# liron88/HM-16.2

Measured on AMD Instinct MI355X. Metric: CTUs/sec (enc) at 4K main10; bit-exact CU partition vs HM, higher is better.
Workload: dtype int32+f64

## Files before the change

__graft_entry__.py:

```python
import os
import subprocess
import sys

ROOT = os.path.dirname(os.path.abspath(__file__))
PKG = os.path.join(ROOT, "hm-16.2_amd")
for p in (ROOT, PKG, os.path.join(ROOT, "oracle")):
    if p not in sys.path:
        sys.path.insert(0, p)


def _newer(target, sources):
    if not os.path.exists(target):
        return True
    t = os.path.getmtime(target)
    return any(os.path.getmtime(s) > t for s in sources)


def build_product():
    src = os.path.join(PKG, "csrc")
    out = os.path.join(PKG, "libhm355.so")
    deps = [os.path.join(src, f) for f in ("hm355.hip", "hm355_core.h", "hm355_inter.h", "hm355_inter_cu.h", "hm355_dbk.h", "hm355_sao.h", "hm355_bits.h", "hm355_bits_kernel.h", "hm355_ingest.h", "hm355_picstat.h", "hm355_types.h", "hm355_host_common.h", "hm355_simt.h", "hm355_simt4.h", "hm355_simt8.h", "hm355_simt16.h", "hm355_team.h")] + [os.path.join(ROOT, "include", "hm355.h")]
    if _newer(out, deps):
        import hashlib
        h = hashlib.sha1()
        for d in sorted(deps):
            h.update(open(d, "rb").read())
        build_id = h.hexdigest()[:12]
        hipcc = "/opt/rocm/bin/hipcc" if os.path.exists("/opt/rocm/bin/hipcc") else "hipcc"
        cmd = [hipcc, "-O3", "--offload-arch=gfx950", "-ffp-contract=off", "-fPIC", "-shared", "-std=c++17", "-Wno-unused-value", "-Wno-sizeof-array-div",
               f'-DHM355_BUILD_ID="{build_id}"', "-o", out, os.path.join(src, "hm355.hip")]
        subprocess.run(cmd, check=True)
    host = os.path.join(PKG, "host")
    exe = os.path.join(PKG, "hm355_encmain")
    if _newer(exe, [os.path.join(host, f) for f in ("encmain.cpp", "TEncTop.cpp", "TEncTop.h")] + [out]):
        subprocess.run(["g++", "-O2", "-std=c++14", "-Wall", "-o", exe, os.path.join(host, "encmain.cpp"), os.path.join(host, "TEncTop.cpp"),
                        "-L" + PKG, "-lhm355", "-Wl,-rpath,$ORIGIN"], check=True)
    return out


def build_oracle():
    subprocess.run(["make", "-s", "-C", os.path.join(ROOT, "oracle"),
                    os.path.join(ROOT, "oracle", "libhm_oracle.so"), os.path.join(ROOT, "oracle", "hm_oracle_cli")], check=True)
    if os.path.isdir("/root/reference/source"):
        subprocess.run(["make", "-s", "-C", os.path.join(ROOT, "oracle"), "ref"], check=True, stdout=subprocess.DEVNULL)


def build():
    build_product()
    build_oracle()
    import hm355
    hm355.load_library()


def smoke():
# ... 59 lines not shown
```

hm-16.2_amd/csrc/hm355_core.h:

```cpp
#pragma once
#include <stddef.h>
#include "hm355_types.h"

#ifdef HM355_HOSTSIM
#include <string.h>
#include <math.h>
#include <stdlib.h>
#define HM_DEV static
#define HM_FINL static inline
#define HM_FINL_M inline
#define HM_LAMBDA_INL
#define HM_NOINLINE __attribute__((noinline))
#define HM_CONST static const
#define HM_ASSUME_LDS(p) ((void)0)
#define HM_ASSUME_GLB(p) ((void)0)
#define HM_NT 1
static inline int hm_lane() { return 0; }
#define HM_SYNC() ((void)0)
static inline uint32_t hm_wave_sum(uint32_t v) { return v; }
static inline int hm_wave_sum_i(int v) { return v; }
static inline int hm_wave_max_i(int v) { return v; }
#define HM_UNI(x) (x)
#define HM_UCALL(x) (x)
#define hm_uni_ptr(p) (p)
// ... 65 lines not shown
{
  static_assert(sizeof(T) % 4 == 0, "dword-sized aggregates only");
  int w[sizeof(T) / 4];
  __builtin_memcpy(w, &v, sizeof(T));
#pragma unroll
  for (unsigned i = 0; i < sizeof(T) / 4; i++) w[i] = __builtin_amdgcn_readfirstlane(w[i]);
  __builtin_memcpy(&v, w, sizeof(T));
  return v;
}
#define HM_ENTRY(e) do { (e) = hm_uni_ptr(e); HM_ASSUME_LDS(e); } while (0)
#define HM_UCALL(x) ((uint32_t)__builtin_amdgcn_readfirstlane((int)(x)))
#define HM_PAR_FOR(i, n) for (int i = hm_lane(); i < (n); i += HM_NT)
#define HM_PAR_FOR_XY(x, y, w, n) \
  for (int i_ = hm_lane(), sy_ = HM_NT / (w), sx_ = HM_NT - sy_ * (w), y = i_ / (w), x = i_ - y * (w); i_ < (n); \
       i_ += HM_NT, x += sx_, y += sy_, (x >= (w) ? (x -= (w), y++) : 0))
#define HM_WAVE_FOR(k) for (int k = hm_lane(), k##_once = 1; k##_once; k##_once = 0)
#define HM_LV(T, name) T name
#define HM_LVARG(T, name) const T name
#define HM_LVK(name, k) name
#define HM_LV_GET(name, i) __builtin_amdgcn_readlane((int)(name), (int)(i))
#define HM_LV_GETD(name, i) hm_readlane_d((name), (int)(i))
#define HM_LV_SET(name, i, v) ((name) = (hm_lane() == (int)(i)) ? (v) : (name))
#define HM_LV_SETD(name, i, v) ((name) = (hm_lane() == (int)(i)) ? (v) : (name))
#define HM_LV_GATHER(name, idx) __builtin_amdgcn_ds_bpermute((int)(idx) << 2, (int)(name))
#define HM_BALLOT(m, k, cond) ((m) = __ballot(cond))
#define HM_ORDERED_ADD16(acc, name) do { _Pragma("unroll") for (int k_ = 15; k_ >= 0; k_--) (acc) += hm_readlane_d((name), k_); } while (0)
#define HM_ORDERED_CHAIN16(acc, a, b, pre) do { _Pragma("unroll") for (int k_ = 15; k_ >= 0; k_--) { \
    (pre) = (hm_lane() == k_) ? (acc) : (pre); (acc) -= hm_readlane_d((a), k_); (acc) += hm_readlane_d((b), k_); } } while (0)
__device__ __forceinline__ double hm_readlane_d(double v, int i)
{ return __hiloint2double(__builtin_amdgcn_readlane(__double2hiint(v), i), __builtin_amdgcn_readlane(__double2loint(v), i)); }
#endif

#if defined(HM355_PROFILE) && !defined(HM355_HOSTSIM)
#define HM_PROF_N 45
#define HM_PROF_BEGIN(e, id) const unsigned long long prof_t0_##id = __builtin_readcyclecounter()
#define HM_PROF_END(e, id) do { (e)->prof[id] += __builtin_readcyclecounter() - prof_t0_##id; (e)->profCnt[id] += 1; } while (0)
#else
#define HM_PROF_BEGIN(e, id) ((void)0)
#define HM_PROF_END(e, id) ((void)0)
#endif
enum { PR_RDOQ = 0, PR_BITS, PR_ADI, PR_PRED, PR_FWD, PR_INV, PR_SATD35, PR_TUBLK, PR_SAVE, PR_CHROMA, PR_LUMA, PR_ENCCU, PR_TOTAL,
       PR_S4L = 32, PR_S4C, PR_D0, PR_D1, PR_D2, PR_D3, PR_NXN, PR_S8L, PR_S4LEAF, PR_S4CLEAF, PR_S8C, PR_S16L = 44,
       PR_ME_INT = 16, PR_ME_FRAC, PR_AMVP, PR_MRG_EST, PR_MC, PR_IRQ, PR_IRES, PR_MRG2N, PR_INTERCU, PR_INTRA_IN_P, PR_IQ_FULL, PR_IQ_FWD, PR_IQ_RDOQ, PR_IQ_BITS, PR_IQ_INV, PR_IQ_ENC };

#define HM_MAX_DOUBLE 1.7e+308
#define PLANAR_IDX 0
#define DC_IDX 1
#define HOR_IDX 10
#define VER_IDX 26
#define DM_CHROMA_IDX 36
#define SIZE_2Nx2N 0
#define SIZE_NxN 3
#define SIZE_NONE 8
#define MODE_INTRA 1
#define MODE_NONE 2
#define SCAN_DIAG 0
#define SCAN_HOR 1
#define SCAN_VER 2

HM_CONST uint8_t HM_NEXT_LPS[128] __attribute__((aligned(4))) = {
  1, 0, 0, 1, 2, 3, 4, 5, 4, 5, 8, 9, 8, 9, 10, 11, 12, 13, 14, 15, 16, 17, 18, 19, 18, 19, 22, 23, 22, 23, 24, 25,
  26, 27, 26, 27, 30, 31, 30, 31, 32, 33, 32, 33, 36, 37, 36, 37, 38, 39, 38, 39, 42, 43, 42, 43, 44, 45, 44, 45, 46, 47, 48, 49,
  48, 49, 50, 51, 52, 53, 52, 53, 54, 55, 54, 55, 56, 57, 58, 59, 58, 59, 60, 61, 60, 61, 60, 61, 62, 63, 64, 65, 64, 65, 66, 67,
  66, 67, 66, 67, 68, 69, 68, 69, 70, 71, 70, 71, 70, 71, 72, 73, 72, 73, 72, 73, 74, 75, 74, 75, 74, 75, 76, 77, 76, 77, 126, 127 };
HM_CONST int32_t HM_ENTROPY_BITS[128] = {
  0x07b23, 0x085f9, 0x074a0, 0x08cbc, 0x06ee4, 0x09354, 0x067f4, 0x09c1b, 0x060b0, 0x0a62a, 0x05a9c, 0x0af5b, 0x0548d, 0x0b955, 0x04f56, 0x0c2a9,
  0x04a87, 0x0cbf7, 0x045d6, 0x0d5c3, 0x04144, 0x0e01b, 0x03d88, 0x0e937, 0x039e0, 0x0f2cd, 0x03663, 0x0fc9e, 0x03347, 0x10600, 0x03050, 0x10f95,
  0x02d4d, 0x11a02, 0x02ad3, 0x12333, 0x0286e, 0x12cad, 0x02604, 0x136df, 0x02425, 0x13f48, 0x021f4, 0x149c4, 0x0203e, 0x1527b, 0x01e4d, 0x15d00,
  0x01c99, 0x166de, 0x01b18, 0x17017, 0x019a5, 0x17988, 0x01841, 0x18327, 0x016df, 0x18d50, 0x015d9, 0x19547, 0x0147c, 0x1a083, 0x0138e, 0x1a8a3,
  0x01251, 0x1b418, 0x01166, 0x1bd27, 0x01068, 0x1c77b, 0x00f7f, 0x1d18e, 0x00eda, 0x1d91a, 0x00e19, 0x1e254, 0x00d4f, 0x1ec9a, 0x00c90, 0x1f6e0,
  0x00c01, 0x1fef8, 0x00b5f, 0x208b1, 0x00ab6, 0x21362, 0x00a15, 0x21e46, 0x00988, 0x2285d, 0x00934, 0x22ea8, 0x008a8, 0x239b2, 0x0081d, 0x24577,
  0x007c9, 0x24ce6, 0x00763, 0x25663, 0x00710, 0x25e8f, 0x006a0, 0x26a26, 0x00672, 0x26f23, 0x005e8, 0x27ef8, 0x005ba, 0x284b5, 0x0055e, 0x29057,
  0x0050c, 0x29bab, 0x004c1, 0x2a674, 0x004a7, 0x2aa5e, 0x0046f, 0x2b32f, 0x0041f, 0x2c0ad, 0x003e7, 0x2ca8d, 0x003ba, 0x2d323, 0x0010c, 0x3bfbb };
HM_CONST uint8_t HM_CTX_INIT_I[HM_NUM_CTX] = {
   139, 141, 157,
// ... 1754 lines not shown
        cabac_copy(&e->cur, &e->ws->slot[HM_SLOT(fullDepth, CI_QT_TRAFO_ROOT)]);
        const uint32_t splitBits = HM_UCALL(intra_bits_qt(e, *t, 1, 0));
        f->splitCost = calc_rd_cost(e, splitBits, f->splitDist);
        if (f->splitCost < f->singleCost) { retDist[sp] += f->splitDist; retBits[sp] += splitBits; retCost[sp] += f->splitCost; sp--; continue; }
      }
      cabac_copy(&e->cur, &e->ws->slot[HM_SLOT(fullDepth, CI_QT_TRAFO_TEST)]);
      par_set8(m->tr + z, t->trDepth, t->parts);
      par_set8(m->cbf[0] + z, (int)(f->singleCbf << t->trDepth), t->parts);
      par_set8(m->ts[0] + z, f->bestModeId, t->parts);
      {
        const int n = 1 << log2, layer = 5 - log2, ps = e->stride[0];
        par_copy_blk(e->fb.rec[0] + (e->ctuY * 64 + t->y) * ps + e->ctuX * 64 + t->x, ps, e->ws->qtRec[layer] + t->y * 64 + t->x, 64, n);
      }
      retDist[sp] += f->singleDist; retBits[sp] += f->singleBits; retCost[sp] += f->singleCost; sp--; continue;
    }
  }
  e->outDistY = retDist[0]; e->outRdCost = retCost[0];
}

HM_DEV inline void set_intra_result_qt(Shared *e, const TU *root)
{
  const CtuMeta *m = (&e->meta);
  for (int rel = root->relZ; rel < root->relZ + root->parts;) {
    const int z = root->cuZ + rel, trd = m->tr[z];
    const int log2 = 6 - root->cuDepth - trd, n = 1 << log2, layer = 5 - log2;
    const int parts = root->cuParts >> (2 * trd) > 0 ? root->cuParts >> (2 * trd) : 1;
    const int r = hm_z2r(z), x = (r & 15) * 4, y = (r >> 4) * 4;
    par_copy32(e->cc + z * 16, e->ws->qtCoef[layer] + z * 16, n * n);
    par_copy_blk(e->ws->reco + y * 64 + x, 64, e->ws->qtRec[layer] + y * 64 + x, 64, n);
    rel += parts;
  }
}

#include "hm355_simt.h"
#include "hm355_simt4.h"
#include "hm355_simt8.h"
#include "hm355_simt16.h"

HM_DEV HM_NOINLINE uint32_t est_intra_pred_qt(Shared *e, int cuZ, int cuDepth)
{
  HM_ENTRY(e); cuZ = HM_UNI(cuZ); cuDepth = HM_UNI(cuDepth);
  CtuMeta *m = (&e->meta); WorkSpace *ws = e->ws;
  const int cuParts = 256 >> (2 * cuDepth);
  const int nxn = m->part[cuZ] == SIZE_NxN;
  const int numPU = nxn ? 4 : 1, puParts = cuParts / numPU;
  const int puLog2 = 6 - cuDepth - nxn, n = 1 << puLog2;
  const int bitDepth = e->bitDepth, ps = e->stride[0];
  uint32_t overallDistY = 0;
  const TU root = tu_root(e, cuZ, cuDepth);
  for (int pu = 0; pu < numPU; pu++) {
    const TU t = nxn ? tu_child(&root, pu, 0) : root;
    const int z = cuZ + t.relZ;
    int numModesForFullRD = HM_INTRA_MODE_NUM_FAST[puLog2 - 1];
    int32_t *rdModeList = e->rdModeList;
    {
      const int r = hm_z2r(z);
      init_adi_pattern(e, 0, e->ctuX * 64 + t.x, e->ctuY * 64 + t.y, n, e->ctuX * 16 + (r & 15), e->ctuY * 16 + (r >> 4), n / 4, 1);
      const Pel *org = e->fb.org[0] + (e->ctuY * 64 + t.y) * ps + e->ctuX * 64 + t.x;
      Pel *pred = ws->pred + t.y * 64 + t.x;
      int preds[3];
      const int numMpm = intra_dir_predictor(e, z, preds);
      e->mpmZ = z; e->mpmNum = numMpm; e->mpmPreds[0] = preds[0]; e->mpmPreds[1] = preds[1]; e->mpmPreds[2] = preds[2];
      const uint64_t frac0 = e->ws->slot[HM_SLOT(cuDepth, CI_CURR_BEST)].frac & 32767;
      const uint8_t st0 = e->ws->slot[HM_SLOT(cuDepth, CI_CURR_BEST)].s[C_INTRA_LUMA];
      HM_PROF_BEGIN(e, PR_SATD35);
      if (n <= 16) satd_all_modes_small(e, org, ps, n);
      else {
        for (int mode = 0; mode < 35; mode++) {
          pred_intra(e, 0, mode, n, use_filtered_refs(0, mode, n), pred, 64);
          const uint32_t sad = dist_hads(org, ps, pred, 64, n, bitDepth);
// ... 106 lines not shown
      const int isOne = (total == 1), isLast = (currModeId == total);
      const uint32_t distTmp = HM_UCALL(intra_coding_tu_block(e, *t, comp, isOne ? 0 : (tsMode == 0 ? 1 : 2)));
      const uint32_t cbfTmp = (m->cbf[comp][zc] >> t->trDepth) & 1;
      if (tsMode == 1 && cbfTmp == 0) costTmp = HM_MAX_DOUBLE;
      else if (!isOne) { reset_bits(&e->cur); enc_coeff_qt(e, t, comp); costTmp = calc_rd_cost(e, num_bits(&e->cur), distTmp); }
      if (costTmp < singleCost) {
        singleCost = costTmp; singleDistC = distTmp; bestTS = tsMode; bestModeId = currModeId; singleCbfC = cbfTmp;
        if (!isOne && !isLast) { store_intra_result_qt(e, t, comp); cabac_copy(&e->ws->slot[HM_SLOT(fullDepth, CI_TEMP_BEST)], &e->cur); }
      }
      if (!isOne && !isLast) cabac_copy(&e->cur, &e->ws->slot[HM_SLOT(fullDepth, CI_QT_TRAFO_ROOT)]);
    }
    if (bestModeId < total) {
      load_intra_result_qt(e, t, comp);
      par_set8(m->cbf[comp] + zc, (int)(singleCbfC << t->trDepth), t->cParts);
      cabac_copy(&e->cur, &e->ws->slot[HM_SLOT(fullDepth, CI_TEMP_BEST)]);
    }
    par_set8(m->ts[comp] + zc, bestTS, t->cParts);
    dist += singleDistC;
  }
  return dist;
}
HM_DEV HM_NOINLINE uint32_t recur_intra_chroma_coding_qt(Shared *e, TU rootv)
{
  HM_ENTRY(e); rootv = hm_uni_struct(rootv);
  const TU *root = &rootv;
  CtuMeta *m = (&e->meta);
  uint32_t dist = 0;
  tu_walk(e->walkOuter, root, 0,
    [&](const TU *t) {
      if (m->tr[t->cuZ + t->relZ] != t->trDepth) return 1;
      if (t->cW) dist += chroma_tu(e, t);
      return 0;
    },
    [&](const TU *t) {
      const int z = t->cuZ + t->relZ, q = t->parts >> 2;
      int any = 0;
      for (int c = 1; c < 3; c++) for (int s = 0; s < 4; s++) any |= ((m->cbf[c][z + s * q] >> (t->trDepth + 1)) & 1) << c;
      HM_PAR_FOR(o, t->parts) for (int c = 1; c < 3; c++) if ((any >> c) & 1) m->cbf[c][z + o] |= (uint8_t)(1 << t->trDepth);
      HM_SYNC();
    });
  return dist;
}
HM_DEV inline void set_intra_result_chroma_qt(Shared *e, const TU *root)
{
  const CtuMeta *m = (&e->meta);
  tu_walk(e->walkOuter, root, 0, [&](const TU *t) {
    if (!t->cW) return 0;
    if (m->tr[t->cuZ + t->relZ] != t->trDepth) return 1;
    const int n = t->cW, layer = 5 - t->log2;
    for (int c = 1; c < 3; c++) {
      const int po = HM_PLANE_OFF(c);
      par_copy32(e->cc + po + t->cOff, e->ws->qtCoef[layer] + po + t->cOff, n * n);
      par_copy_blk(e->ws->reco + po + t->cy * 32 + t->cx, 32, e->ws->qtRec[layer] + po + t->cy * 32 + t->cx, 32, n);
    }
    return 0;
  });
}
HM_DEV HM_NOINLINE uint32_t est_intra_pred_chroma_qt(Shared *e, int cuZ, int cuDepth)
{
  HM_ENTRY(e); cuZ = HM_UNI(cuZ); cuDepth = HM_UNI(cuDepth);
  CtuMeta *m = (&e->meta); WorkSpace *ws = e->ws; const int cuParts = 256 >> (2 * cuDepth);
  const TU t = tu_root(e, cuZ, cuDepth);
  if (cuDepth == 3) {
    const int split = m->tr[cuZ] != 0;
    int tsLuma = 0;
    if (split) for (int s = 0; s < 4; s++) tsLuma += m->ts[0][cuZ + s];
    if (!tsLuma) {
      cabac_copy(&e->cur, &e->ws->slot[HM_SLOT(cuDepth, CI_CURR_BEST)]);
      HM_PROF_BEGIN(e, PR_S4C);
      const uint32_t d = HM_UCALL(simt4_chroma_cu(e, split ? tu_child(&t, 0, 0) : t, cuZ));
      HM_PROF_END(e, PR_S4C);
      cabac_copy(&e->cur, &e->ws->slot[HM_SLOT(cuDepth, CI_CURR_BEST)]);
      return d;
    }
  }
  if (cuDepth == 2) {
    int split = 0;
    for (int i = 0; i < 16; i += 4) split |= m->tr[cuZ + i];
    if (!split) {
      cabac_copy(&e->cur, &e->ws->slot[HM_SLOT(cuDepth, CI_CURR_BEST)]);
      HM_PROF_BEGIN(e, PR_S8C);
      const uint32_t d = HM_UCALL(simt8_chroma_cu16(e, cuZ));
      HM_PROF_END(e, PR_S8C);
      cabac_copy(&e->cur, &e->ws->slot[HM_SLOT(cuDepth, CI_CURR_BEST)]);
      return d;
    }
  }
  int bestMode = 0; uint32_t bestDist = 0; double bestCost = HM_MAX_DOUBLE;
  int modeList[5];
  allowed_chroma_dirs(m->dirL[cuZ], modeList);
  for (int mi = 0; mi < 5; mi++) {
    cabac_copy(&e->cur, &e->ws->slot[HM_SLOT(cuDepth, CI_CURR_BEST)]);
    par_set8(m->dirC + cuZ, modeList[mi], cuParts);
    const uint32_t dist = HM_UCALL(recur_intra_chroma_coding_qt(e, t));
    cabac_copy(&e->cur, &e->ws->slot[HM_SLOT(cuDepth, CI_CURR_BEST)]);
    const uint32_t bits = HM_UCALL(intra_bits_qt(e, t, 0, 1));
    const double cost = calc_rd_cost(e, bits, dist);
    if (cost < bestCost) {
      bestCost = cost; bestDist = dist; bestMode = modeList[mi];
      set_intra_result_chroma_qt(e, &t);
      HM_PAR_FOR(i, cuParts) for (int c = 1; c < 3; c++) { ws->saveCbf[c][i] = m->cbf[c][cuZ + i]; ws->saveTs[c][i] = m->ts[c][cuZ + i]; }
      HM_SYNC();
    }
  }
  HM_PAR_FOR(i, cuParts) { for (int c = 1; c < 3; c++) { m->cbf[c][cuZ + i] = ws->saveCbf[c][i]; m->ts[c][cuZ + i] = ws->saveTs[c][i]; } m->dirC[cuZ + i] = (uint8_t)bestMode; }
  HM_SYNC();
  cabac_copy(&e->cur, &e->ws->slot[HM_SLOT(cuDepth, CI_CURR_BEST)]);
  return bestDist;
}

template <class C> HM_DEV inline void code_delta_qp(Shared *e, C *c, int dqp)
{
  const int off = 6 * (e->bitDepth - 8);
  dqp = (dqp + 78 + off + (off / 2)) % (52 + off) - 26 - (off / 2);
  const uint32_t a = (uint32_t)hm_abs(dqp), tu = a < 5 ? a : 5;
  enc_bin(e, c, C_DQP, tu ? 1 : 0);
  if (tu) { for (uint32_t k = tu; --k;) enc_bin(e, c, C_DQP + 1, 1); if (5 > tu) enc_bin(e, c, C_DQP + 1, 0); }
  if (a >= 5) {
    uint32_t sym = a - 5, count = 0, bins = 0; int nb = 0;
    while (sym >= (1u << count)) { bins = 2 * bins + 1; nb++; sym -= 1u << count; count++; }
    bins = 2 * bins; nb++;
    bins = (bins << count) | sym; nb += (int)count;
    enc_epv(c, bins, nb);
  }
  if (a > 0) enc_epv(c, dqp > 0 ? 0u : 1u, 1);
}
template <class C> HM_DEV inline void code_dqp_if_due(Shared *e, C *c)
{
  if (!e->fb.dqp) return;
  WorkSpace *ws = e->ws;
  if (!HM_UNI(ws->dq.flag)) return;
  code_delta_qp(e, c, HM_UNI(ws->dq.ctuQp) - HM_UNI(ws->dq.refQp));
  HM_SYNC();
  if (hm_lane() == 0) ws->dq.flag = 0;
  HM_SYNC();
}
HM_DEV inline void check_dqp(Shared *e, int cuZ, int cuDepth)
{
  if (!e->fb.dqp || cuDepth != 0) return;
  const CtuMeta *m = &e->meta;
// ... 379 lines not shown
```

hm-16.2_amd/csrc/hm355_simt.h:

```cpp
#pragma once

template <int L2> struct SimtDim {
  enum { NC = 1 << (2 * L2), NCG = NC / 16, WCG = 1 << (L2 - 2), NSIG = L2 == 2 ? 9 : (L2 == 3 ? 21 : 27), NSET = NCG == 1 ? 1 : 4, NGRP = 2 * L2, NCGC = NCG == 1 ? 0 : 2,
         NLAST = L2 == 4 ? 4 : 3, LSH = L2 == 4 ? 1 : L2 - 2,
         X_SIG = 0, X_ONE = NSIG, X_ABS = X_ONE + 4 * NSET, X_LX = X_ABS + NSET, X_LY = X_LX + NLAST, X_CG = X_LY + NLAST, X_CBF = X_CG + NCGC,
         X_MODE = X_CBF + 1, X_TSKIP = X_MODE + 1, NCTX = X_TSKIP + (L2 == 2 ? 1 : 0),
         T_SIG = 0, T_ONE = 2 * NSIG, T_ABS = T_ONE + 8 * NSET, T_LASTX = T_ABS + 2 * NSET, T_LASTY = T_LASTX + NGRP, T_CG = T_LASTY + NGRP,
         T_CBF = T_CG + 2 * NCGC, T_N = T_CBF + 2 };
};
static_assert(SimtDim<2>::NCTX == 23 && SimtDim<2>::T_N == 38 && SimtDim<2>::X_LX == 14 && SimtDim<2>::X_LY == 17 && SimtDim<2>::X_CBF == 20 && SimtDim<2>::T_LASTX == 28 &&
              SimtDim<2>::T_LASTY == 32 && SimtDim<2>::T_CBF == 36 && SimtDim<2>::LSH == 0, "the 4x4 batch's numbering");
static_assert(SimtDim<3>::NCTX == 51 && SimtDim<3>::T_N == 100 && SimtDim<3>::X_ONE == 21 && SimtDim<3>::X_ABS == 37 && SimtDim<3>::X_LX == 41 && SimtDim<3>::X_LY == 44 &&
              SimtDim<3>::X_CG == 47 && SimtDim<3>::X_CBF == 49 && SimtDim<3>::T_ONE == 42 && SimtDim<3>::T_ABS == 74 && SimtDim<3>::T_LASTX == 82 && SimtDim<3>::T_LASTY == 88 &&
              SimtDim<3>::T_CG == 94 && SimtDim<3>::T_CBF == 98 && SimtDim<3>::LSH == 1 && SimtDim<3>::WCG == 2, "the 8x8 batch's numbering");
template <int L2> struct Simt;
template <int L2> struct SimtPrices {
  const int32_t *tab;
  HM_FINL_M int one(int i) const { return tab[SimtDim<L2>::T_ONE + i]; }
  HM_FINL_M int abs2(int i) const { return tab[SimtDim<L2>::T_ABS + i]; }
};

struct SimtPar {
  int chroma, bitDepth, qBits, quantCoef, tshift; double errScale, lambda; int64_t rdFactor;
  int dqShift, dqScale, dqMin, dqMax;
// ... 8 lines not shown
  int tgt = 25 + p.dqShift; if (tgt > 16) tgt = 16;
  p.dqMin = -(1 << (tgt - 1)); p.dqMax = (1 << (tgt - 1)) - 1;
  return p;
}
HM_FINL int32_t simt_level_double(int sc, const SimtPar &p)
{
  const int64_t cap = 2147483647LL - (1LL << (p.qBits - 1));
  const int64_t tl = (int64_t)hm_abs(sc) * p.quantCoef;
  return (int32_t)(tl < cap ? tl : cap);
}
HM_FINL int simt_dequant(const SimtPar &p, int level)
{
  const int c = hm_clip3(p.dqMin, p.dqMax, level);
  int v;
  if (p.dqShift > 0) v = (c * p.dqScale + (1 << (p.dqShift - 1))) >> p.dqShift;
  else v = (int)((unsigned)(c * p.dqScale) << (-p.dqShift));
  return hm_clip3(-32768, 32767, v);
}

template <int L2> HM_FINL int simt_ctx_index(int j, int chroma, int cbfCodeCtx, int modeCtx)
{
  typedef SimtDim<L2> D;
  const int lastOff = chroma ? 15 : 3 * (L2 - 2);
  if (j < D::X_ONE) return C_SIG + (chroma ? 28 : 0) + (chroma && j >= 16 ? 0 : j);
  if (j < D::X_ABS) return C_ONE + (chroma ? 16 + ((j - D::X_ONE) & 7) : j - D::X_ONE);
  if (j < D::X_LX) return C_ABS + (chroma ? 4 + ((j - D::X_ABS) & 1) : j - D::X_ABS);
  if (j < D::X_LY) return C_LASTX + lastOff + (j - D::X_LX);
  if (j < D::X_CG) return C_LASTY + lastOff + (j - D::X_LY);
  if (j < D::X_CBF) return C_SIG_CG + (chroma ? 2 : 0) + (j - D::X_CG);
  if (j == D::X_CBF) return C_QT_CBF + cbfCodeCtx;
  if (j == D::X_MODE) return modeCtx;
  return C_TSKIP + (chroma ? 1 : 0);
}
template <int L2> HM_DEV inline void simt_setup(Shared *e, const Simt<L2> &S, const Cabac *cb, int jobs, int chroma, int cbfCtx, int cbfCodeCtx, int modeCtx)
{
  typedef SimtDim<L2> D;
  HM_PAR_FOR(i, D::T_N) {
    const int bin = i & 1;
    int v = 0;
    if (i < D::T_LASTX) {
      const int j = i >> 1, none = chroma && ((j < D::X_ONE && j >= 16) || (j >= D::X_ONE && j < D::X_ABS && j - D::X_ONE >= 8) || (j >= D::X_ABS && j - D::X_ABS >= 2));
      if (!none) v = HM_LT()->ebits[cb->s[simt_ctx_index<L2>(j, chroma, 0, 0)] ^ bin];
    } else if (i < D::T_CG) {
      const int g = (i - D::T_LASTX) % D::NGRP, x0 = i < D::T_LASTY ? D::X_LX : D::X_LY;
      for (int c = 0; c < g; c++) v += HM_LT()->ebits[cb->s[simt_ctx_index<L2>(x0 + (c >> D::LSH), chroma, 0, 0)] ^ 1];
      if (g < D::NGRP - 1) v += HM_LT()->ebits[cb->s[simt_ctx_index<L2>(x0 + (g >> D::LSH), chroma, 0, 0)] ^ 0];
      if (g > 3) v += 32768 * ((g - 2) >> 1);
    } else if (i < D::T_CBF) v = HM_LT()->ebits[cb->s[simt_ctx_index<L2>(D::X_CG + ((i - D::T_CG) >> 1), chroma, 0, 0)] ^ bin];
    else v = HM_LT()->ebits[cb->s[C_QT_CBF + cbfCtx] ^ bin];
    S.tab()[i] = v;
  }
  HM_PAR_FOR(i, 128) S.lps()[i] = HM_NEXT_LPS[i];
  HM_PAR_FOR(i, D::NCTX * S.JOBS) {
    const int j = i / S.JOBS, k = i - j * S.JOBS;
    if (k < jobs) S.ctx(j, k) = cb->s[simt_ctx_index<L2>(j, chroma, cbfCodeCtx, modeCtx)];
  }
  S.load_scans(e);
  HM_SYNC();
}
template <int L2> HM_FINL void simt_store_contexts(const Simt<L2> &S, int k, Cabac *cb, int cbfCodeCtx)
{
  HM_PAR_FOR(j, SimtDim<L2>::NCTX) cb->s[simt_ctx_index<L2>(j, 0, cbfCodeCtx, C_INTRA_LUMA)] = S.ctx(j, k);
}

template <int L2> HM_DEV inline void simt_bin(const Shared *e, const Simt<L2> &S, int k, uint32_t *frac, int c, int bin)
{
  const int st = S.ctx(c, k);
  *frac += (uint32_t)HM_LT()->ebits[st ^ bin];
  S.ctx(c, k) = (uint8_t)(bin == (st & 1) ? (st < 124 ? st + 2 : st) : S.lps()[st]);
}
template <int L2> HM_FINL int simt_cg_pattern(int cgBlkPos, int cgMask)
{
  const int W = SimtDim<L2>::WCG, cgx = cgBlkPos & (W - 1), cgy = cgBlkPos >> (L2 - 2);
  const int sigRight = cgx < W - 1 ? ((cgMask >> (cgBlkPos + 1)) & 1) : 0, sigLower = cgy < W - 1 ? ((cgMask >> (cgBlkPos + W)) & 1) : 0;
  return sigRight + (sigLower << 1);
}
template <int L2> HM_FINL void simt_last_xy(int blkPos, int scanType, int *px, int *py)
{
  const int y = blkPos >> L2, x = blkPos & ((1 << L2) - 1);
// ... 156 lines not shown
              if (lastCG == 1 && lastNZ == q && hm_abs(dv) == 1) costDown -= (4 << 15);
              if (costUp < costDown) { curCost = costUp; curChange = 1; }
              else { curChange = -1; if (q == firstNZ && hm_abs(dv) == 1) curCost = I64MAX; else curCost = costDown; }
            } else {
              curCost = p.rdFactor * (-(hm_abs(deltaU))) + (1 << 15) + rateIncUp + sigRateDelta;
              curChange = 1;
              if (q < firstNZ) { const uint32_t thissign = sc < 0 ? 1u : 0u; if (thissign != signbit) curCost = I64MAX; }
            }
            if (curCost < minCostInc) { minCostInc = curCost; finalChange = curChange; minK = q; }
          }
          if (minK >= 0) {
            int mv = S.lev(subPos + minK, k);
            if (mv == 32767 || mv == -32768) finalChange = -1;
            mv = (S.cs(subPos + minK, k) < 0) ? mv - finalChange : mv + finalChange;
            S.put_lev(subPos + minK, k, mv);
          }
        }
      }
      if (lastCG == 1) lastCG = 0;
    }
  }
  return absSum;
}

template <int L2> HM_DEV inline void simt_code_coeff(const Shared *e, const Simt<L2> &S, int k, int src, int chroma, int scanType, uint32_t *frac)
{
  typedef SimtDim<L2> D;
  int last = -1, cgMask = 0;
  for (int sp = 0; sp < D::NC; sp++)
    if (S.lev(sp, src) != 0) { last = sp; cgMask |= 1 << S.cg_pos(scanType, sp >> 4); }
  {
    int px, py; simt_last_xy<L2>(S.scan_pos(scanType, last), scanType, &px, &py);
    const int gx = hm_group_idx(px), gy = hm_group_idx(py);
    int q;
    for (q = 0; q < gx; q++) simt_bin(e, S, k, frac, D::X_LX + (q >> D::LSH), 1);
    if (gx < D::NGRP - 1) simt_bin(e, S, k, frac, D::X_LX + (q >> D::LSH), 0);
    for (q = 0; q < gy; q++) simt_bin(e, S, k, frac, D::X_LY + (q >> D::LSH), 1);
    if (gy < D::NGRP - 1) simt_bin(e, S, k, frac, D::X_LY + (q >> D::LSH), 0);
    if (gx > 3) *frac += 32768u * (uint32_t)((gx - 2) >> 1);
    if (gy > 3) *frac += 32768u * (uint32_t)((gy - 2) >> 1);
  }
  const int firstCtx = first_sig_ctx(1 << L2, scanType, chroma), lastSet = last >> 4;
  int c1 = 1;
  for (int subSet = lastSet; subSet >= 0; subSet--) {
    const int subPos = subSet << 4, isLastSet = subSet == lastSet;
    const int cgBlkPos = S.cg_pos(scanType, subSet), pattern = simt_cg_pattern<L2>(cgBlkPos, cgMask);
    if (isLastSet || subSet == 0) cgMask |= 1 << cgBlkPos;
    else simt_bin(e, S, k, frac, D::X_CG + (pattern != 0), (cgMask >> cgBlkPos) & 1);
    if (!((cgMask >> cgBlkPos) & 1)) continue;
    const int top = isLastSet ? (last & 15) : 15;
    int numNonZero = isLastSet ? 1 : 0, firstNZ = isLastSet ? top : 16, lastNZ = isLastSet ? top : -1;
    for (int q = isLastSet ? top - 1 : 15; q >= 0; q--) {
      const int sig = S.lev(subPos + q, src) != 0;
      if (q > 0 || subSet == 0 || numNonZero) simt_bin(e, S, k, frac, D::X_SIG + S.sig_inc(scanType, firstCtx, pattern, subPos + q, chroma), sig);
      if (sig) { numNonZero++; firstNZ = q; if (lastNZ < 0) lastNZ = q; }
    }
    if (numNonZero > 0) {
      const int signHidden = (lastNZ - firstNZ >= 4);
      const int ctxSet = ((subSet > 0 && !chroma) ? 2 : 0) + (c1 == 0 ? 1 : 0);
      c1 = 1;
      int firstC2 = -1, escape = 0, idx = 0;
      for (int q = lastNZ; q >= 0 && idx < 8; q--) {
        const int a = hm_abs(S.lev(subPos + q, src));
        if (!a) continue;
        const int sym = a > 1;
        simt_bin(e, S, k, frac, D::X_ONE + 4 * ctxSet + c1, sym);
        if (sym) { c1 = 0; if (firstC2 == -1) firstC2 = q; else escape = 1; }
        else if (c1 < 3 && c1 > 0) c1++;
        idx++;
      }
      if (c1 == 0 && firstC2 != -1) { const int sym = hm_abs(S.lev(subPos + firstC2, src)) > 2; simt_bin(e, S, k, frac, D::X_ABS + ctxSet, sym); if (sym) escape = 1; }
// ... 42 lines not shown
```

hm-16.2_amd/csrc/hm355_types.h:

```cpp
#pragma once
#include <stdint.h>

typedef int16_t Pel;
typedef int32_t TCoeff;

enum {
  C_SPLIT = 0, C_PART = 3, C_INTRA_LUMA = 7, C_CHROMA_PRED = 8, C_SUBDIV = 10, C_QT_CBF = 13, C_SIG_CG = 23,
  C_SIG = 27, C_LASTX = 71, C_LASTY = 101, C_ONE = 131, C_ABS = 155, C_TSKIP = 161,
   C_SKIP = 163, C_MRG_FLAG = 166, C_MRG_IDX = 167, C_PRED_MODE = 168, C_INTER_DIR = 169, C_MVD = 174, C_REF = 176,
  C_ROOT_CBF = 178, C_MVP_IDX = 179,  C_DQP = 180, HM_NUM_CTX = 183
};
struct Cabac {
  uint8_t s[184];
  uint64_t frac;
};
enum { CI_CURR_BEST = 0, CI_NEXT_BEST, CI_TEMP_BEST, CI_QT_TRAFO_TEST, CI_QT_TRAFO_ROOT, CI_NUM };

struct CtuMeta {
  uint8_t depth[256], part[256], pred[256], dirL[256], dirC[256], tr[256], cbf[3][256], ts[3][256];
};
struct CtuStat { double cost; uint32_t bits, dist; };
struct MvD { int16_t x, y; };
struct InterMeta {
  uint8_t skip[256], mrg[256], mrgIdx[256], interDir[256];
// ... 27 lines not shown
struct Best {
  CtuMeta m;
  InterMeta im;
  TCoeff coef[HM_COEF_CTU];
  Pel reco[HM_COEF_CTU];
};

struct WorkSpace {
  Best best[4];
  Pel pred[HM_COEF_CTU], resi[HM_COEF_CTU], reco[HM_COEF_CTU];
  Pel qtRec[4][HM_COEF_CTU];
  TCoeff qtCoef[4][HM_COEF_CTU];
  MvD intMv[2][16];
  Pel tsPred[3][16], tsRec[3][16]; TCoeff tsCoef[3][16];
  double costCoeff[1024];
  Cabac slot[4 * CI_NUM + 3];
  Pel tmpPred[HM_COEF_CTU];
  Pel resiBest[HM_COEF_CTU];
  Pel mcTmp[72 * 64];
  Pel mcBlk[64 * 64];
  Pel yuvPred[2][HM_COEF_CTU];
  Pel orgBi[64 * 64];
  struct PuSearch {
    MvD mvTemp[2][16], mvPred[2][16], mvPredBi[2][16], cand[2][16][2];
    int8_t mvpIdx[2][16], mvpIdxBi[2][16], mvpNum[2][16];
    uint32_t costTempL0[16], bitsTempL0[16];
  } ps;
  struct { MvD mv[5][2]; int32_t ref[5][2]; uint8_t dir[5]; int32_t num; } mrg2N;
  uint8_t tmpTr[256], tmpCbf[3][256], tmpTs[3][256], saveCbf[3][256], saveTs[3][256];
  struct { int32_t ctuQp, refQp, flag, pad; } dq;
  TCoeff teamCoef[HM_COEF_CTU];
  InterMeta teamIm;
  MvD teamTok[3][2][16];
};

struct QpTab { int32_t qpPer[2], qpRem[2]; double errScale[2][4]; int64_t rdFactor[2]; };
struct CtuDqp {
  int8_t qp, refQp, lastQp;
  uint8_t flagOut;
  int16_t firstZ, pad;
};
struct CtuRc {
  double lambda, sqrtLambda, lambdaC;
  int64_t rdFactor[2];
  uint32_t lambdaMotionSAD, lambdaMotionSSE;
};
struct CtuRcOut { int32_t bits, qp; };
struct DqpPic {
  int32_t flagIn, sliceQp;
  const int8_t *ctuQp;
  CtuDqp *out;
  const uint8_t *rowFlag;
  QpTab tab[64];
  const CtuRc *rc;
  CtuRcOut *rcOut;
  int32_t firstCtu, pad;
};

struct Tables {
  uint8_t z2r[256], r2z[256];
  uint16_t scan[3][4][1024];
  uint16_t scanCG[3][4][64];
};

struct FrameBuf {
  Pel *org[3], *rec[3];
// ... 33 lines not shown
```

Before: 25850.

## Batch chroma intra mode search across modes with SIMT leaf transforms

Adds a SIMT chroma path for depth-0/1 CUs whose transform trees use only 16x16 or 8x8 chroma TUs. All five chroma modes for both planes are processed as parallel jobs per leaf, with per-mode reconstruction, coefficients and CBFs kept in new workspace buffers. For one tree class the rate is estimated lane-parallel, one lane per mode, instead of a serial CABAC pass per mode. This adds workspace memory and new code paths, and it relies on the SIMT rate model staying bit-exact with the existing chroma RD search. It also fixes the last-position context shift used for 16x16 chroma.

```diff
diff --git a/__graft_entry__.py b/__graft_entry__.py
--- a/__graft_entry__.py
+++ b/__graft_entry__.py
@@ -19,7 +19,7 @@
 def build_product():
     src = os.path.join(PKG, "csrc")
     out = os.path.join(PKG, "libhm355.so")
-    deps = [os.path.join(src, f) for f in ("hm355.hip", "hm355_core.h", "hm355_inter.h", "hm355_inter_cu.h", "hm355_dbk.h", "hm355_sao.h", "hm355_bits.h", "hm355_bits_kernel.h", "hm355_ingest.h", "hm355_picstat.h", "hm355_types.h", "hm355_host_common.h", "hm355_simt.h", "hm355_simt4.h", "hm355_simt8.h", "hm355_simt16.h", "hm355_team.h")] + [os.path.join(ROOT, "include", "hm355.h")]
+    deps = [os.path.join(src, f) for f in ("hm355.hip", "hm355_core.h", "hm355_inter.h", "hm355_inter_cu.h", "hm355_dbk.h", "hm355_sao.h", "hm355_bits.h", "hm355_bits_kernel.h", "hm355_ingest.h", "hm355_picstat.h", "hm355_types.h", "hm355_host_common.h", "hm355_simt.h", "hm355_simt4.h", "hm355_simt8.h", "hm355_simt16.h", "hm355_simt_chroma.h", "hm355_team.h")] + [os.path.join(ROOT, "include", "hm355.h")]
     if _newer(out, deps):
         import hashlib
         h = hashlib.sha1()
diff --git a/hm-16.2_amd/csrc/hm355_core.h b/hm-16.2_amd/csrc/hm355_core.h
--- a/hm-16.2_amd/csrc/hm355_core.h
+++ b/hm-16.2_amd/csrc/hm355_core.h
@@ -121,7 +121,7 @@
 #endif
 
 #if defined(HM355_PROFILE) && !defined(HM355_HOSTSIM)
-#define HM_PROF_N 45
+#define HM_PROF_N 50
 #define HM_PROF_BEGIN(e, id) const unsigned long long prof_t0_##id = __builtin_readcyclecounter()
 #define HM_PROF_END(e, id) do { (e)->prof[id] += __builtin_readcyclecounter() - prof_t0_##id; (e)->profCnt[id] += 1; } while (0)
 #else
@@ -129,7 +129,7 @@
 #define HM_PROF_END(e, id) ((void)0)
 #endif
 enum { PR_RDOQ = 0, PR_BITS, PR_ADI, PR_PRED, PR_FWD, PR_INV, PR_SATD35, PR_TUBLK, PR_SAVE, PR_CHROMA, PR_LUMA, PR_ENCCU, PR_TOTAL,
-       PR_S4L = 32, PR_S4C, PR_D0, PR_D1, PR_D2, PR_D3, PR_NXN, PR_S8L, PR_S4LEAF, PR_S4CLEAF, PR_S8C, PR_S16L = 44,
+       PR_S4L = 32, PR_S4C, PR_D0, PR_D1, PR_D2, PR_D3, PR_NXN, PR_S8L, PR_S4LEAF, PR_S4CLEAF, PR_S8C, PR_S16L = 44, PR_SCHROMA, PR_CHROMA_FB, PR_CHROMA_CLS ,
        PR_ME_INT = 16, PR_ME_FRAC, PR_AMVP, PR_MRG_EST, PR_MC, PR_IRQ, PR_IRES, PR_MRG2N, PR_INTERCU, PR_INTRA_IN_P, PR_IQ_FULL, PR_IQ_FWD, PR_IQ_RDOQ, PR_IQ_BITS, PR_IQ_INV, PR_IQ_ENC };
 
 #define HM_MAX_DOUBLE 1.7e+308
@@ -1950,10 +1950,21 @@
   }
 }
 
+HM_FINL void chroma_cbf_of_split_node(Shared *e, const TU *t)
+{
+  CtuMeta *m = (&e->meta);
+  const int z = t->cuZ + t->relZ, q = t->parts >> 2;
+  int any = 0;
+  for (int c = 1; c < 3; c++) for (int s = 0; s < 4; s++) any |= ((m->cbf[c][z + s * q] >> (t->trDepth + 1)) & 1) << c;
+  HM_PAR_FOR(o, t->parts) for (int c = 1; c < 3; c++) if ((any >> c) & 1) m->cbf[c][z + o] |= (uint8_t)(1 << t->trDepth);
+  HM_SYNC();
+}
+
 #include "hm355_simt.h"
 #include "hm355_simt4.h"
 #include "hm355_simt8.h"
 #include "hm355_simt16.h"
+#include "hm355_simt_chroma.h"
 
 HM_DEV HM_NOINLINE uint32_t est_intra_pred_qt(Shared *e, int cuZ, int cuDepth)
 {
@@ -2126,13 +2137,7 @@
       if (t->cW) dist += chroma_tu(e, t);
       return 0;
     },
-    [&](const TU *t) {
-      const int z = t->cuZ + t->relZ, q = t->parts >> 2;
-      int any = 0;
-      for (int c = 1; c < 3; c++) for (int s = 0; s < 4; s++) any |= ((m->cbf[c][z + s * q] >> (t->trDepth + 1)) & 1) << c;
-      HM_PAR_FOR(o, t->parts) for (int c = 1; c < 3; c++) if ((any >> c) & 1) m->cbf[c][z + o] |= (uint8_t)(1 << t->trDepth);
-      HM_SYNC();
-    });
+    [&](const TU *t) { chroma_cbf_of_split_node(e, t); });
   return dist;
 }
 HM_DEV inline void set_intra_result_chroma_qt(Shared *e, const TU *root)
@@ -2180,6 +2185,24 @@
       return d;
     }
   }
+  const int cls = cuDepth <= 1 ? simt_chroma_tree_class(e, cuZ, cuDepth) : 0;
+#if defined(HM355_PROFILE) && !defined(HM355_HOSTSIM)
+  const unsigned long long clsT0 = __builtin_readcyclecounter();
+#define HM_PROF_CHROMA_CLS() do { if (cls) { e->prof[PR_CHROMA_CLS + cls - 1] += __builtin_readcyclecounter() - clsT0; e->profCnt[PR_CHROMA_CLS + cls - 1] += 1; } } while (0)
+#else
+#define HM_PROF_CHROMA_CLS() ((void)0)
+#endif
+  if (cls && ((HM355_SCHROMA_CLASSES >> (cls - 1)) & 1)) {
+    HM_PROF_BEGIN(e, PR_SCHROMA);
+    const uint32_t d = HM_UCALL(simt_chroma_cu(e, cuZ, cuDepth, cls));
+    HM_PROF_END(e, PR_SCHROMA);
+    HM_PROF_CHROMA_CLS();
+    return d;
+  }
+#ifdef HM355_HOSTSIM
+  g_schroma_stats.fallback[cuDepth]++;
+#endif
+  HM_PROF_BEGIN(e, PR_CHROMA_FB);
   int bestMode = 0; uint32_t bestDist = 0; double bestCost = HM_MAX_DOUBLE;
   int modeList[5];
   allowed_chroma_dirs(m->dirL[cuZ], modeList);
@@ -2200,6 +2223,8 @@
   HM_PAR_FOR(i, cuParts) { for (int c = 1; c < 3; c++) { m->cbf[c][cuZ + i] = ws->saveCbf[c][i]; m->ts[c][cuZ + i] = ws->saveTs[c][i]; } m->dirC[cuZ + i] = (uint8_t)bestMode; }
   HM_SYNC();
   cabac_copy(&e->cur, &e->ws->slot[HM_SLOT(cuDepth, CI_CURR_BEST)]);
+  HM_PROF_END(e, PR_CHROMA_FB);
+  HM_PROF_CHROMA_CLS();
   return bestDist;
 }
 
diff --git a/hm-16.2_amd/csrc/hm355_simt.h b/hm-16.2_amd/csrc/hm355_simt.h
--- a/hm-16.2_amd/csrc/hm355_simt.h
+++ b/hm-16.2_amd/csrc/hm355_simt.h
@@ -64,6 +64,7 @@
   if (j == D::X_MODE) return modeCtx;
   return C_TSKIP + (chroma ? 1 : 0);
 }
+template <int L2> HM_FINL int simt_last_shift(int chroma) { return (L2 == 4 && chroma) ? 2 : (int)SimtDim<L2>::LSH; }
 template <int L2> HM_DEV inline void simt_setup(Shared *e, const Simt<L2> &S, const Cabac *cb, int jobs, int chroma, int cbfCtx, int cbfCodeCtx, int modeCtx)
 {
   typedef SimtDim<L2> D;
@@ -74,9 +75,9 @@
       const int j = i >> 1, none = chroma && ((j < D::X_ONE && j >= 16) || (j >= D::X_ONE && j < D::X_ABS && j - D::X_ONE >= 8) || (j >= D::X_ABS && j - D::X_ABS >= 2));
       if (!none) v = HM_LT()->ebits[cb->s[simt_ctx_index<L2>(j, chroma, 0, 0)] ^ bin];
     } else if (i < D::T_CG) {
-      const int g = (i - D::T_LASTX) % D::NGRP, x0 = i < D::T_LASTY ? D::X_LX : D::X_LY;
-      for (int c = 0; c < g; c++) v += HM_LT()->ebits[cb->s[simt_ctx_index<L2>(x0 + (c >> D::LSH), chroma, 0, 0)] ^ 1];
-      if (g < D::NGRP - 1) v += HM_LT()->ebits[cb->s[simt_ctx_index<L2>(x0 + (g >> D::LSH), chroma, 0, 0)] ^ 0];
+      const int g = (i - D::T_LASTX) % D::NGRP, x0 = i < D::T_LASTY ? D::X_LX : D::X_LY, lsh = simt_last_shift<L2>(chroma);
+      for (int c = 0; c < g; c++) v += HM_LT()->ebits[cb->s[simt_ctx_index<L2>(x0 + (c >> lsh), chroma, 0, 0)] ^ 1];
+      if (g < D::NGRP - 1) v += HM_LT()->ebits[cb->s[simt_ctx_index<L2>(x0 + (g >> lsh), chroma, 0, 0)] ^ 0];
       if (g > 3) v += 32768 * ((g - 2) >> 1);
     } else if (i < D::T_CBF) v = HM_LT()->ebits[cb->s[simt_ctx_index<L2>(D::X_CG + ((i - D::T_CG) >> 1), chroma, 0, 0)] ^ bin];
     else v = HM_LT()->ebits[cb->s[C_QT_CBF + cbfCtx] ^ bin];
@@ -299,11 +300,11 @@
   {
     int px, py; simt_last_xy<L2>(S.scan_pos(scanType, last), scanType, &px, &py);
     const int gx = hm_group_idx(px), gy = hm_group_idx(py);
-    int q;
-    for (q = 0; q < gx; q++) simt_bin(e, S, k, frac, D::X_LX + (q >> D::LSH), 1);
-    if (gx < D::NGRP - 1) simt_bin(e, S, k, frac, D::X_LX + (q >> D::LSH), 0);
-    for (q = 0; q < gy; q++) simt_bin(e, S, k, frac, D::X_LY + (q >> D::LSH), 1);
-    if (gy < D::NGRP - 1) simt_bin(e, S, k, frac, D::X_LY + (q >> D::LSH), 0);
+    int q; const int lsh = simt_last_shift<L2>(chroma);
+    for (q = 0; q < gx; q++) simt_bin(e, S, k, frac, D::X_LX + (q >> lsh), 1);
+    if (gx < D::NGRP - 1) simt_bin(e, S, k, frac, D::X_LX + (q >> lsh), 0);
+    for (q = 0; q < gy; q++) simt_bin(e, S, k, frac, D::X_LY + (q >> lsh), 1);
+    if (gy < D::NGRP - 1) simt_bin(e, S, k, frac, D::X_LY + (q >> lsh), 0);
     if (gx > 3) *frac += 32768u * (uint32_t)((gx - 2) >> 1);
     if (gy > 3) *frac += 32768u * (uint32_t)((gy - 2) >> 1);
   }
diff --git a/hm-16.2_amd/csrc/hm355_simt_chroma.h b/hm-16.2_amd/csrc/hm355_simt_chroma.h
--- /dev/null
+++ b/hm-16.2_amd/csrc/hm355_simt_chroma.h
@@ -0,0 +1,260 @@
+#pragma once
+
+#ifdef HM355_HOSTSIM
+struct SimtChromaStats {
+  unsigned long taken[2][3], batches16, batches8, leaves16, leaves8, fallback[4];
+  ~SimtChromaStats()
+  {
+    if (!getenv("HM355_SCHROMA_STATS")) return;
+    fprintf(stderr, "schroma taken"); for (int i = 0; i < 6; i++) fprintf(stderr, " %lu", taken[i / 3][i % 3]);
+    fprintf(stderr, "\nschroma batches %lu %lu leaves %lu %lu", batches16, batches8, leaves16, leaves8);
+    fprintf(stderr, "\nschroma fallback"); for (int i = 0; i < 4; i++) fprintf(stderr, " %lu", fallback[i]);
+    fprintf(stderr, "\n");
+  }
+};
+static SimtChromaStats g_schroma_stats;
+#endif
+
+#ifndef HM355_SCHROMA_CLASSES
+#define HM355_SCHROMA_CLASSES 6
+#endif
+HM_FINL int simt_chroma_tree_class(const Shared *e, int cuZ, int cuDepth)
+{
+  const CtuMeta *m = (&e->meta);
+  const int tr16 = 1 - cuDepth;
+  int seen = 0;
+  HM_PAR_FOR(i, 64 >> (2 * cuDepth)) {
+    const int d = m->tr[cuZ + 4 * i] - tr16;
+    seen |= d == 0 ? 1 : (d == 1 ? 2 : 4);
+  }
+  seen = hm_wave_max_i(seen & 4) | hm_wave_max_i(seen & 2) | hm_wave_max_i(seen & 1);
+  return (seen & 4) ? 0 : seen;
+}
+
+HM_FINL int sc_line_off(int n, int j) { return n == 16 ? (j < 3 ? 33 * (j + 1) : 165 + 33 * (j - 3)) : (j < 5 ? 17 * (j + 1) : 149 + 17 * (j - 5)); }
+static_assert(165 + 33 + 33 <= 264 && 149 + 4 * 17 + 17 <= 264 && 5 * 17 + 17 <= 132 && 3 * 33 + 33 <= 132, "four line sets of 33 or ten of 17 beside the builder's");
+HM_FINL int sc_dc_val(const Pel *top, const Pel *left, int n)
+{
+  int s = 0;
+  HM_PAR_FOR(i, n) s += top[i + 1] + left[i + 1];
+  return (hm_wave_sum_i(s) + n) / (n + n);
+}
+template <class Pred> HM_FINL void sn_residual_fwd(const Simt8 &S, const Pel *org, int ps, int bitDepth, int job, Pred pred) { s8_residual_fwd(S, org, ps, bitDepth, SCAN_DIAG, job, pred); }
+template <class Pred> HM_FINL void sn_residual_fwd(const Simt16 &S, const Pel *org, int ps, int bitDepth, int job, Pred pred) { s16_residual_fwd(S, org, ps, bitDepth, job, pred); }
+
+HM_FINL void sc_build_lines(Shared *e, const TU *t, const TU *root, int m0, int m1)
+{
+  WorkSpace *ws = e->ws;
+  const int n = t->cW, r = hm_z2r(t->cuZ + t->relZ);
+  const int x4 = e->ctuX * 16 + (r & 15), y4 = e->ctuY * 16 + (r >> 4), px = e->ctuX * 32 + t->cx, py = e->ctuY * 32 + t->cy;
+  const int first = t->relZ == 0;
+  Pel *topF = &e->u.ref.refTop[0][0], *leftF = &e->u.ref.refLeft[0][0];
+  for (int mi = m0; mi < m1; mi++) {
+    if (!first) {
+      for (int c = 0; c < 2; c++) {
+        Pel *rec = e->fb.rec[1 + c]; const int st = e->stride[1 + c]; const Pel *own = ws->chRec[mi] + c * 1024;
+        HM_PAR_FOR(i, 4 * n + 1) {
+          const int cx = i <= 2 * n ? t->cx - 1 + i : t->cx - 1, cy = i <= 2 * n ? t->cy - 1 : t->cy + (i - 2 * n - 1);
+          if (cx >= root->cx && cx < root->cx + root->cW && cy >= root->cy && cy < root->cy + root->cW)
+            rec[(e->ctuY * 32 + cy) * st + e->ctuX * 32 + cx] = own[cy * 32 + cx];
+        }
+      }
+      HM_SYNC();
+    }
+    if (!first || mi == 0) simt_chroma_ref_lines(e, px, py, n, x4, y4);
+    HM_PAR_FOR(i, 2 * (2 * n + 1)) {
+      const int c = i > 2 * n, k = i - c * (2 * n + 1), o = sc_line_off(n, 2 * (mi - m0) + c) + k;
+      topF[o] = e->u.ref.refTop[c][k]; leftF[o] = e->u.ref.refLeft[c][k];
+    }
+    HM_SYNC();
+  }
+}
+
+template <int L2> HM_FINL int sc_job_is_empty(const Simt<L2> &S, const SimtPar &p, int job)
+{
+  int mx = 0;
+  HM_PAR_FOR(l, 1 << (2 * L2)) { const int a = hm_abs(S.cs(l, job)); mx = a > mx ? a : mx; }
+  mx = hm_wave_max_i(mx);
+  return ((simt_level_double(mx, p) + (1 << (p.qBits - 1))) >> p.qBits) == 0;
+}
+template <int L2> HM_FINL void sc_leaf(Shared *e, const TU *t, const TU *root, const int *modeList, int lumaDir)
+{
+  enum { N = 1 << L2, MB = L2 == 3 ? 5 : HM_S16 / 2 };
+  WorkSpace *ws = e->ws;
+  const Simt<L2> S(e);
+  const int bitDepth = e->bitDepth, shiftSse = (bitDepth - 8) << 1;
+  const int px = e->ctuX * 32 + t->cx, py = e->ctuY * 32 + t->cy;
+  const Pel *topF = &e->u.ref.refTop[0][0], *leftF = &e->u.ref.refLeft[0][0];
+  const SimtPar p = simt_params<L2>(e, 1);
+  for (int m0 = 0; m0 < 5; m0 += MB) {
+    const int m1 = m0 + MB < 5 ? m0 + MB : 5, nj = 2 * (m1 - m0);
+    sc_build_lines(e, t, root, m0, m1);
+    if (m0 == 0) simt_setup(e, S, &e->cur, 0, 1, 5 + t->trDepth, 5 + t->trDepth, C_CHROMA_PRED);
+    int live = 0;
+    for (int job = 0; job < nj; job++) {
+      const int c = job & 1, dirC = chroma_mode_at(modeList, m0 + (job >> 1)), mode = dirC == DM_CHROMA_IDX ? lumaDir : dirC, ps = e->stride[1 + c];
+      const Pel *top = topF + sc_line_off(N, job), *left = leftF + sc_line_off(N, job);
+      const int dcVal = mode == DC_IDX ? sc_dc_val(top, left, N) : 0;
+      sn_residual_fwd(S, e->fb.org[1 + c] + (size_t)py * ps + px, ps, bitDepth, job,
+                      [&](int x, int y) HM_LAMBDA_INL { return intra_pred_sample(top, left, N, L2, 0, mode, x, y, dcVal, 0); });
+      if (!sc_job_is_empty(S, p, job)) live |= 1 << job;
+    }
+    HM_WAVE_FOR(k) { if (k < nj) sn_out_cbf(S)[k] = (uint8_t)(((live >> k) & 1) && simt_rdoq(S, p, k, SCAN_DIAG) > 0); }
+    HM_SYNC();
+    for (int job = 0; job < nj; job++) {
+      const int c = job & 1, mi = m0 + (job >> 1), dirC = chroma_mode_at(modeList, mi), mode = dirC == DM_CHROMA_IDX ? lumaDir : dirC, ps = e->stride[1 + c];
+      const int cbf = HM_UNI(sn_out_cbf(S)[job]);
+      const Pel *top = topF + sc_line_off(N, job), *left = leftF + sc_line_off(N, job);
+      const int dcVal = mode == DC_IDX ? sc_dc_val(top, left, N) : 0;
+      const Pel *org = e->fb.org[1 + c] + (size_t)py * ps + px;
+      Pel *own = ws->chRec[mi] + c * 1024 + t->cy * 32 + t->cx;
+      sn_dequant_inv1(S, p, job, cbf, ws->chCoef[mi] + c * 1024 + t->cOff, SCAN_DIAG);
+      uint32_t sse = 0;
+      sn_inv2_recon(S, bitDepth, cbf, [&](int x, int y) HM_LAMBDA_INL { return intra_pred_sample(top, left, N, L2, 0, mode, x, y, dcVal, 0); },
+                    [&](int x, int y, int rr) HM_LAMBDA_INL { const int d = org[y * ps + x] - rr; sse += (uint32_t)((d * d) >> shiftSse); own[y * 32 + x] = (Pel)rr; });
+      const uint32_t dsum = hm_wave_sum(sse);
+      if (hm_lane() == 0) e->satd[mi] += (uint32_t)(e->fb.chromaWeight * (double)dsum);
+      par_set8(ws->chCbf[mi][c] + t->relZ, cbf << t->trDepth, t->parts);
+    }
+#ifdef HM355_HOSTSIM
+    if (L2 == 4) g_schroma_stats.batches16++; else g_schroma_stats.batches8++;
+#endif
+  }
+#ifdef HM355_HOSTSIM
+  if (L2 == 4) g_schroma_stats.leaves16++; else g_schroma_stats.leaves8++;
+#endif
+}
+
+HM_DEV HM_NOINLINE uint32_t simt_chroma_bits(Shared *e, TU tv, const TCoeff *planes)
+{
+  HM_ENTRY(e); tv = hm_uni_struct(tv); planes = hm_uni_ptr(planes);
+  const TU *root = &tv; const CtuMeta *m = (&e->meta);
+  HM_PROF_BEGIN(e, PR_BITS);
+  {
+    CabacR r; cabr_load(e, r, &e->cur);
+    r.frac &= 32767;
+    enc_intra_header(e, &r, root, 0, 1);
+    enc_subdiv_cbf_qt(e, &r, root, 0, 1);
+    cabr_store(r, &e->cur);
+  }
+  for (int comp = 1; comp < 3; comp++)
+    tu_walk(e->walkInner, root, 0, [&](const TU *t) {
+      if (m->tr[t->cuZ + t->relZ] > t->trDepth) return 1;
+      code_tu_coeff(e, &e->cur, t, comp, planes, 1);
+      return 0;
+    });
+  HM_PROF_END(e, PR_BITS);
+  return num_bits(&e->cur);
+}
+
+template <int L2> HM_FINL void sc_bin_reg(const Simt<L2> &S, int32_t *state, uint32_t *frac, int bin)
+{
+  const int st = *state;
+  *frac += (uint32_t)HM_LT()->ebits[st ^ bin];
+  *state = bin == (st & 1) ? (st < 124 ? st + 2 : st) : S.lps()[st];
+}
+HM_FINL int sc_decide_lanes8(Shared *e, const TU *root, const int *modeList)
+{
+  const CtuMeta *m = (&e->meta); WorkSpace *ws = e->ws;
+  const Simt8 S(e); Simt8A *A = S.A;
+  simt_setup(e, S, &e->cur, 5, 1, 5, 5, C_CHROMA_PRED);
+  const uint32_t baseFrac = (uint32_t)(e->cur.frac & 32767);
+  const int cbfState[3] = { e->cur.s[C_QT_CBF + 5], e->cur.s[C_QT_CBF + 6], e->cur.s[C_QT_CBF + 7] };
+  HM_LV(uint32_t, vFrac); HM_LV(int32_t, vCbf0); HM_LV(int32_t, vCbf1); HM_LV(int32_t, vCbf2);
+  HM_WAVE_FOR(k) {
+    uint32_t frac = baseFrac;
+    if (k < 5) {
+      const int dirC = chroma_mode_at(modeList, k);
+      simt_bin(e, S, k, &frac, SimtDim<3>::X_MODE, dirC != DM_CHROMA_IDX);
+      if (dirC != DM_CHROMA_IDX) frac += 2u * 32768u;
+    }
+    HM_LVK(vFrac, k) = frac; HM_LVK(vCbf0, k) = cbfState[0]; HM_LVK(vCbf1, k) = cbfState[1]; HM_LVK(vCbf2, k) = cbfState[2];
+  }
+  tu_walk(e->walkInner, root, 0, [&](const TU *t) {
+    const int d = t->trDepth;
+    HM_WAVE_FOR(k) {
+      if (k < 5) {
+        uint32_t frac = HM_LVK(vFrac, k); int32_t st = d == 0 ? HM_LVK(vCbf0, k) : (d == 1 ? HM_LVK(vCbf1, k) : HM_LVK(vCbf2, k));
+        for (int c = 0; c < 2; c++) {
+          const int b = ws->chCbf[k][c][t->relZ];
+          if (d == 0 || ((b >> (d - 1)) & 1)) sc_bin_reg(S, &st, &frac, (b >> d) & 1);
+        }
+        HM_LVK(vFrac, k) = frac;
+        if (d == 0) HM_LVK(vCbf0, k) = st; else if (d == 1) HM_LVK(vCbf1, k) = st; else HM_LVK(vCbf2, k) = st;
+      }
+    }
+    return m->tr[t->cuZ + t->relZ] > d;
+  });
+  for (int c = 0; c < 2; c++)
+    tu_walk(e->walkInner, root, 0, [&](const TU *t) {
+      if (m->tr[t->cuZ + t->relZ] > t->trDepth) return 1;
+      HM_PAR_FOR(i, 5 * 64) { const int mi = i >> 6, sp = i & 63; S.put_lev(sp, mi, ws->chCoef[mi][c * 1024 + t->cOff + S.scan_pos(SCAN_DIAG, sp)]); }
+      HM_SYNC();
+      HM_WAVE_FOR(k) {
+        if (k < 5 && ((ws->chCbf[k][c][t->relZ] >> t->trDepth) & 1)) { uint32_t frac = HM_LVK(vFrac, k); simt_code_coeff(e, S, k, k, 1, SCAN_DIAG, &frac); HM_LVK(vFrac, k) = frac; }
+      }
+      HM_SYNC();
+      return 0;
+    });
+  HM_WAVE_FOR(k) { if (k < 5) A->outCost[k] = calc_rd_cost(e, HM_LVK(vFrac, k) >> 15, e->satd[k]); }
+  HM_SYNC();
+  double bestCost = HM_MAX_DOUBLE; int best = 0;
+  for (int mi = 0; mi < 5; mi++) { const double v = A->outCost[mi]; if (v < bestCost) { bestCost = v; best = mi; } }
+  return HM_UNI(best);
+}
+
+HM_DEV HM_NOINLINE uint32_t simt_chroma_cu(Shared *e, int cuZ, int cuDepth, int cls)
+{
+  HM_ENTRY(e); cuZ = HM_UNI(cuZ); cuDepth = HM_UNI(cuDepth); cls = HM_UNI(cls);
+  CtuMeta *m = (&e->meta); WorkSpace *ws = e->ws; const int cuParts = 256 >> (2 * cuDepth);
+  const TU root = tu_root(e, cuZ, cuDepth);
+  const int lumaDir = m->dirL[cuZ];
+  int modeList[5];
+  allowed_chroma_dirs(lumaDir, modeList);
+  cabac_copy(&e->cur, &e->ws->slot[HM_SLOT(cuDepth, CI_CURR_BEST)]);
+  HM_PAR_FOR(i, 5) e->satd[i] = 0;
+  HM_PAR_FOR(i, cuParts) { m->ts[1][cuZ + i] = 0; m->ts[2][cuZ + i] = 0; }
+  HM_SYNC();
+#ifdef HM355_HOSTSIM
+  g_schroma_stats.taken[cuDepth][cls - 1]++;
+#endif
+  tu_walk(e->walkOuter, &root, 0,
+    [&](const TU *t) {
+      if (m->tr[t->cuZ + t->relZ] != t->trDepth) return 1;
+      if (t->cW == 16) sc_leaf<4>(e, t, &root, modeList, lumaDir); else sc_leaf<3>(e, t, &root, modeList, lumaDir);
+      return 0;
+    },
+    [&](const TU *t) {
+      const int q = t->parts >> 2;
+      HM_PAR_FOR(i, 10 * t->parts) {
+        const int a = i / t->parts, o = i - a * t->parts; uint8_t *cb = ws->chCbf[a >> 1][a & 1] + t->relZ;
+        int any = 0;
+        for (int s = 0; s < 4; s++) any |= (cb[s * q] >> (t->trDepth + 1)) & 1;
+        if (any) cb[o] |= (uint8_t)(1 << t->trDepth);
+      }
+      HM_SYNC();
+    });
+  int best = 0;
+  if (cls == 2) best = sc_decide_lanes8(e, &root, modeList);
+  else {
+    double bestCost = HM_MAX_DOUBLE;
+    for (int mi = 0; mi < 5; mi++) {
+      HM_PAR_FOR(i, cuParts) { m->dirC[cuZ + i] = (uint8_t)chroma_mode_at(modeList, mi); m->cbf[1][cuZ + i] = ws->chCbf[mi][0][i]; m->cbf[2][cuZ + i] = ws->chCbf[mi][1][i]; }
+      HM_SYNC();
+      if (mi) cabac_copy(&e->cur, &e->ws->slot[HM_SLOT(cuDepth, CI_CURR_BEST)]);
+      const uint32_t bits = HM_UCALL(simt_chroma_bits(e, root, ws->chCoef[mi] - HM_PLANE_OFF(1)));
+      const double cost = calc_rd_cost(e, bits, HM_UNI(e->satd[mi]));
+      if (cost < bestCost) { bestCost = cost; best = mi; }
+    }
+  }
+  const uint32_t bestDist = HM_UNI(e->satd[best]);
+  HM_PAR_FOR(i, cuParts) { m->cbf[1][cuZ + i] = ws->chCbf[best][0][i]; m->cbf[2][cuZ + i] = ws->chCbf[best][1][i]; m->dirC[cuZ + i] = (uint8_t)chroma_mode_at(modeList, best); }
+  HM_SYNC();
+  for (int c = 1; c < 3; c++) {
+    const int po = HM_PLANE_OFF(c), o = (c - 1) * 1024;
+    par_copy32(e->cc + po + root.cOff, ws->chCoef[best] + o + root.cOff, root.cW * root.cW);
+    par_copy_blk(ws->reco + po + root.cy * 32 + root.cx, 32, ws->chRec[best] + o + root.cy * 32 + root.cx, 32, root.cW);
+  }
+  cabac_copy(&e->cur, &e->ws->slot[HM_SLOT(cuDepth, CI_CURR_BEST)]);
+  return bestDist;
+}
diff --git a/hm-16.2_amd/csrc/hm355_types.h b/hm-16.2_amd/csrc/hm355_types.h
--- a/hm-16.2_amd/csrc/hm355_types.h
+++ b/hm-16.2_amd/csrc/hm355_types.h
@@ -83,6 +83,9 @@
   TCoeff teamCoef[HM_COEF_CTU];
   InterMeta teamIm;
   MvD teamTok[3][2][16];
+  TCoeff chCoef[5][2048];
+  Pel chRec[5][2048];
+  uint8_t chCbf[5][2][256];
 };
 
 struct QpTab { int32_t qpPer[2], qpRem[2]; double errScale[2][4]; int64_t rdFactor[2]; };
```

Result: no change. 25960 (median of 6 runs) (+0.4%).
